# fattorib/ZeRO-transformer

Measured on AMD Instinct MI355X. Metric: training throughput (tokens/s, whole job), higher is better.
Workload: dtype bf16; 1 GPU; model=GPT-1_3b_2048 (1.31B params), global_batch=16, seq_len=2048, train_context=2048, parallelism=dp1+zero1, grad_accum=1

## Files before the change

### zero_transformer_amd/ops/csrc/attention_fwd.hip

```cpp

#include "attn_tiles.h"
#include "common.h"

#include <ATen/ATen.h>
#include <ATen/hip/HIPContext.h>
#include <ATen/hip/impl/HIPStreamMasqueradingAsCUDA.h>
#include <torch/extension.h>

namespace {

using attn::NW;
using attn::RB;
using attn::TB;
using attn::Stage;
using attn::swz;
using attn::tr_frag;

constexpr float NEG_INF = -3.0e38f;

template <int D, int NT, int MINW>
__global__ __launch_bounds__(NT, MINW) void flash_fwd_kernel(
    const uint16_t* __restrict__ qkv, const float* __restrict__ slopes,
    uint16_t* __restrict__ o, float* __restrict__ lse, int H, int T, int C,
    float scale, float p_drop, uint32_t seed) {
  extern __shared__ __attribute__((aligned(16))) char smem[];
  uint16_t* lds0 = (uint16_t*)smem;

  const int bh = blockIdx.x;
  const int h = bh % H;
  const int QS = 3 * C;
  const long base = (long)(bh / H) * T * QS + h * D;
  const long kbase = base + C;
  const long vbase = base + 2 * C;
  const long obase = (long)(bh / H) * T * C + h * D;
  constexpr int RBX = NT / 2;
  const int q0 = blockIdx.y * RBX;
  const int wave = threadIdx.x >> 6;
  const int lane = threadIdx.x & 63;
  const int li = lane & 31;
  const int hi = lane >> 5;
  const int qw = q0 + wave * 32;
  const int qi = qw + li;
  const float slope = slopes[h];
  constexpr float LOG2E = 1.4426950408889634f;
  constexpr float LN2 = 0.6931471805599453f;
  constexpr float DEFER_THR = 11.5f;
  const float scale2 = scale * LOG2E;
  const float slope2 = slope * LOG2E;
  const uint32_t drop_thr = (uint32_t)(p_drop * 256.0f + 0.5f);
  const float inv_keep = drop_thr ? 256.0f / (256.0f - (float)drop_thr) : 1.0f;

  constexpr int KS = D / 16;
  constexpr int DB = D / 32;

  bf16x8 q_frag[KS];
  {
    const bool ok = qi < T;
#pragma unroll
    for (int s = 0; s < KS; ++s)
      q_frag[s] = ok ? *reinterpret_cast<const bf16x8*>(
                           &qkv[base + (long)qi * QS + s * 16 + 8 * hi])
                     : bf16x8{};
  }

  float m_run = NEG_INF, l_run = 0.f;
  f32x16 o_acc[DB];
#pragma unroll
  for (int d = 0; d < DB; ++d) o_acc[d] = f32x16{};

  if (NT == 512 && __builtin_amdgcn_readfirstlane(threadIdx.x) >= 256)
    __builtin_amdgcn_s_setprio(1);

  attn::glds_stage<D, NT / 64>(qkv, kbase, QS, 0, T, lds0);
  attn::glds_stage<D, NT / 64>(qkv, vbase, QS, 0, T, lds0 + TB * 128);
  const int kv_end = min(T, q0 + RBX);
  for (int kt = 0; kt < kv_end; kt += TB) {
    const int cur = (kt / TB) & 1;
    const uint16_t* k_lds = lds0 + (cur ? 2 * TB * 128 : 0);
    const uint16_t* v_lds = lds0 + TB * 128 + (cur ? 2 * TB * 128 : 0);
    __syncthreads();
    attn::lds_acquire();
    if (kt + TB < kv_end) {
      uint16_t* nxt = lds0 + (cur ? 0 : 2 * TB * 128);
      attn::glds_stage<D, NT / 64>(qkv, kbase, QS, kt + TB, T, nxt);
      attn::glds_stage<D, NT / 64>(qkv, vbase, QS, kt + TB, T, nxt + TB * 128);
    }

#pragma unroll
    for (int sub = 0; sub < 2; ++sub) {
      const int kt32 = kt + sub * 32;
      if (kt32 > qw + 31 || kt32 >= T) continue;

      f32x16 s_acc{};
#pragma unroll
      for (int s = 0; s < KS; ++s) {
        const int kk = s * 16 + 8 * hi;
        const int krow = sub * 32 + li;
        bf16x8 a_frag = *reinterpret_cast<const bf16x8*>(
            (char*)k_lds + swz(krow, krow * 256 + kk * 2));
        s_acc = __builtin_amdgcn_mfma_f32_32x32x16_bf16(a_frag, q_frag[s], s_acc, 0, 0, 0);
      }

      float sv_[16];
      float tile_max = NEG_INF;
#pragma unroll
      for (int r = 0; r < 16; ++r) {
        const int kj = kt32 + (r & 3) + 8 * (r >> 2) + 4 * hi;
        float x = s_acc[r] * scale2 + slope2 * (float)(kj - qi);
        if (kj > qi || kj >= T || qi >= T) x = NEG_INF;
        sv_[r] = x;
        tile_max = fmaxf(tile_max, x);
      }
      tile_max = fmaxf(tile_max, __shfl_xor(tile_max, 32, 64));

      float alpha = 1.f;
      const bool valid = tile_max > 0.5f * NEG_INF;
      if (!__all(tile_max <= m_run + DEFER_THR)) {
        const float mn = valid ? fmaxf(m_run, tile_max) : m_run;
        alpha = (m_run > 0.5f * NEG_INF) ? exp2f(m_run - mn) : (valid ? 0.f : 1.f);
        m_run = mn;
      }
      float p[16];
      float row_sum = 0.f;
#pragma unroll
      for (int r = 0; r < 16; ++r) {
        p[r] = (valid && m_run > 0.5f * NEG_INF) ? exp2f(sv_[r] - m_run) : 0.f;
        row_sum += p[r];
      }
      row_sum += __shfl_xor(row_sum, 32, 64);
      l_run = l_run * alpha + row_sum;

      if (drop_thr) {
        const int bhT_qi = bh * T + qi;
#pragma unroll
        for (int g = 0; g < 4; ++g) {
          const int kbase = kt32 + 8 * g + 4 * hi;
          const uint32_t bits = drop_bits32(seed, bhT_qi, kbase >> 2);
#pragma unroll
          for (int e = 0; e < 4; ++e) {
            const bool keep = ((bits >> (8 * e)) & 0xffu) >= drop_thr;
            p[4 * g + e] = keep ? p[4 * g + e] * inv_keep : 0.f;
          }
        }
      }

      if (!__all(alpha == 1.f)) {
#pragma unroll
        for (int r = 0; r < 16; ++r) {
          const float ar = __shfl(alpha, (r & 3) + 8 * (r >> 2) + 4 * hi, 64);
#pragma unroll
          for (int d = 0; d < DB; ++d) o_acc[d][r] *= ar;
        }
      }

      bf16x8 pa[2];
      attn::c_to_a_frags(p, pa);

      attn::TrPair vp[2];
      attn::tr_pair_issue(v_lds, sub * 32, 0, &vp[0]);
#pragma unroll
      for (int d = 0; d < DB; ++d) {
        if (d + 1 < DB) attn::tr_pair_issue(v_lds, sub * 32, (d + 1) * 32, &vp[(d + 1) & 1]);
        attn::TrPair& t = vp[d & 1];
        if (d + 1 < DB)
          attn::tr_pair_wait<4>(&t);
        else
          attn::tr_pair_wait<0>(&t);
        o_acc[d] = __builtin_amdgcn_mfma_f32_32x32x16_bf16(pa[0], t.a, o_acc[d], 0, 0, 0);
        o_acc[d] = __builtin_amdgcn_mfma_f32_32x32x16_bf16(pa[1], t.b, o_acc[d], 0, 0, 0);
      }
    }
  }

  const float inv_l = l_run > 0.f ? 1.f / l_run : 0.f;
  if (hi == 0 && qi < T)
    lse[(long)bh * T + qi] = l_run > 0.f ? m_run * LN2 + __logf(l_run) : NEG_INF;
#pragma unroll
  for (int r = 0; r < 16; ++r) {
    const int row = (r & 3) + 8 * (r >> 2) + 4 * hi;
    const int qr = qw + row;
    if (qr >= T) continue;
    const float il = __shfl(inv_l, row, 64);
#pragma unroll
    for (int d = 0; d < DB; ++d)
      o[obase + (long)qr * C + d * 32 + li] = f32_to_bf16(o_acc[d][r] * il);
  }
}

template <int D>
void launch_fwd(const at::Tensor& qkv, const at::Tensor& slopes, at::Tensor& o,
                at::Tensor& lse, int B, int H, int T, int C, float scale,
                float p_drop, uint32_t seed, hipStream_t stream) {
  const size_t smem = 4 * TB * 128 * sizeof(uint16_t);
  static const bool f4 = [] {
    const char* e = getenv("ZTA_FWD4");
    return e && e[0] == '1';
  }();
  if (f4) {
    dim3 grid(B * H, (T + 127) / 128);
    hipLaunchKernelGGL((flash_fwd_kernel<D, 256, 1>), grid, dim3(256), smem, stream,
                       (const uint16_t*)qkv.data_ptr(), slopes.data_ptr<float>(),
                       (uint16_t*)o.data_ptr(), lse.data_ptr<float>(), H, T, C,
                       scale, p_drop, seed);
    return;
  }
  dim3 grid(B * H, (T + RB - 1) / RB);
  hipLaunchKernelGGL((flash_fwd_kernel<D, 512, 2>), grid, dim3(512), smem, stream,
                     (const uint16_t*)qkv.data_ptr(), slopes.data_ptr<float>(),
                     (uint16_t*)o.data_ptr(), lse.data_ptr<float>(), H, T, C,
                     scale, p_drop, seed);
}

}

std::vector<at::Tensor> attn_fwd(at::Tensor qkv, at::Tensor slopes, int64_t H_,
                                 double p_drop, int64_t seed) {
  TORCH_CHECK(qkv.is_cuda() && qkv.is_contiguous() && qkv.dim() == 3,
              "qkv must be (B, T, 3C) contiguous");
  TORCH_CHECK(qkv.scalar_type() == at::kBFloat16, "attn_fwd: bf16 only");
  const int B = qkv.size(0), T = qkv.size(1), H = (int)H_;
  const int C = qkv.size(2) / 3;
  TORCH_CHECK(qkv.size(2) == 3 * C && C % H == 0, "bad qkv shape");
  const int D = C / H;
  auto o = at::empty({B, T, C}, qkv.options());
  auto lse = at::empty({B, H, T}, qkv.options().dtype(at::kFloat));
  auto sl = slopes.to(at::kFloat).contiguous();
  const float scale = 1.0f / sqrtf((float)D);
  auto stream = at::hip::getCurrentHIPStreamMasqueradingAsCUDA();
  switch (D) {
    case 32: launch_fwd<32>(qkv, sl, o, lse, B, H, T, C, scale, (float)p_drop, (uint32_t)seed, stream); break;
    case 64: launch_fwd<64>(qkv, sl, o, lse, B, H, T, C, scale, (float)p_drop, (uint32_t)seed, stream); break;
    case 96: launch_fwd<96>(qkv, sl, o, lse, B, H, T, C, scale, (float)p_drop, (uint32_t)seed, stream); break;
    case 128: launch_fwd<128>(qkv, sl, o, lse, B, H, T, C, scale, (float)p_drop, (uint32_t)seed, stream); break;
    default: TORCH_CHECK(false, "attn_fwd: head_dim must be one of 32/64/96/128, got ", D);
  }
  return {o, lse};
}
```

### zero_transformer_amd/ops/csrc/attn_tiles.h

```cpp
#pragma once

#include "common.h"

typedef __attribute__((ext_vector_type(8))) __bf16 bf16x8;
typedef __attribute__((ext_vector_type(2))) int i32x2;

#if defined(__HIP_DEVICE_COMPILE__) && defined(__clang_major__)
#if __clang_major__ < 19 || __clang_major__ > 22
#error \
    "attn_tiles.h counted s_waitcnt contracts validated only for ROCm LLVM 19-22; \
re-run tests/test_gpu_ops.py on this compiler and extend the guard (or build \
with -DZTA_SAFE_WAITS=1)."
#endif
#endif
#ifndef ZTA_SAFE_WAITS
#define ZTA_SAFE_WAITS 0
#endif

namespace attn {

constexpr int NW = 8;
constexpr int RB = NW * 32;
constexpr int TB = 64;

ZTA_DEV int swz(int row, int byte_off) { return byte_off ^ ((row & 7) << 4); }

ZTA_DEV void lds_acquire() { asm volatile("" ::: "memory"); }

ZTA_DEV bf16x8 tr_frag(const uint16_t* lds, int k0, int j0) {
  const int l = threadIdx.x & 63;
  const int colb = (j0 + (l & 16) + 4 * (l & 3)) * 2;
  const int r0 = k0 + 8 * (l >> 5) + ((l >> 2) & 3);
  const int a0 = (int)(size_t)((const char*)lds + r0 * 256 + (colb ^ ((r0 & 7) << 4)));
  const int r1 = r0 + 4;
  const int a1 = (int)(size_t)((const char*)lds + r1 * 256 + (colb ^ ((r1 & 7) << 4)));
  union {
    i32x2 d[2];
    bf16x8 v;
  } u;
  asm volatile(
      "ds_read_b64_tr_b16 %0, %2\n\t"
      "ds_read_b64_tr_b16 %1, %3\n\t"
      "s_waitcnt lgkmcnt(0)"
      : "=&v"(u.d[0]), "=&v"(u.d[1])
      : "v"(a0), "v"(a1));
  return u.v;
}

struct TrPair {
  bf16x8 a, b;
};

struct TrQuad {
  TrPair x, y;
};
ZTA_DEV TrQuad tr_frag_quad(const uint16_t* lds_x, const uint16_t* lds_y, int k0,
                            int j0) {
  const int l = threadIdx.x & 63;
  const int colb = (j0 + (l & 16) + 4 * (l & 3)) * 2;
  const int rb = 8 * (l >> 5) + ((l >> 2) & 3);
  int ax[4], ay[4];
#pragma unroll
  for (int i = 0; i < 4; ++i) {
    const int row = k0 + 16 * (i >> 1) + 4 * (i & 1) + rb;
    const int off = row * 256 + (colb ^ ((row & 7) << 4));
    ax[i] = (int)(size_t)((const char*)lds_x + off);
    ay[i] = (int)(size_t)((const char*)lds_y + off);
  }
  union {
    i32x2 d[8];
    TrQuad f;
  } u;
  asm volatile(
      "ds_read_b64_tr_b16 %0, %8\n\t"
      "ds_read_b64_tr_b16 %1, %9\n\t"
      "ds_read_b64_tr_b16 %2, %10\n\t"
      "ds_read_b64_tr_b16 %3, %11\n\t"
      "ds_read_b64_tr_b16 %4, %12\n\t"
      "ds_read_b64_tr_b16 %5, %13\n\t"
      "ds_read_b64_tr_b16 %6, %14\n\t"
      "ds_read_b64_tr_b16 %7, %15\n\t"
      "s_waitcnt lgkmcnt(0)"
      : "=&v"(u.d[0]), "=&v"(u.d[1]), "=&v"(u.d[2]), "=&v"(u.d[3]),
        "=&v"(u.d[4]), "=&v"(u.d[5]), "=&v"(u.d[6]), "=&v"(u.d[7])
      : "v"(ax[0]), "v"(ax[1]), "v"(ax[2]), "v"(ax[3]), "v"(ay[0]), "v"(ay[1]),
        "v"(ay[2]), "v"(ay[3]));
  return u.f;
}
ZTA_DEV void tr_quad_issue(const uint16_t* lds_x, const uint16_t* lds_y, int k0,
                           int j0, TrQuad* out, int l = threadIdx.x & 63) {
  const int colb = (j0 + (l & 16) + 4 * (l & 3)) * 2;
  const int rb = 8 * (l >> 5) + ((l >> 2) & 3);
  int ax[4], ay[4];
#pragma unroll
  for (int i = 0; i < 4; ++i) {
    const int row = k0 + 16 * (i >> 1) + 4 * (i & 1) + rb;
    const int off = row * 256 + (colb ^ ((row & 7) << 4));
    ax[i] = (int)(size_t)((const char*)lds_x + off);
    ay[i] = (int)(size_t)((const char*)lds_y + off);
  }
  union U {
    i32x2 d[8];
    TrQuad f;
  }* u = (union U*)out;
  asm volatile(
      "ds_read_b64_tr_b16 %0, %8\n\t"
      "ds_read_b64_tr_b16 %1, %9\n\t"
      "ds_read_b64_tr_b16 %2, %10\n\t"
      "ds_read_b64_tr_b16 %3, %11\n\t"
      "ds_read_b64_tr_b16 %4, %12\n\t"
      "ds_read_b64_tr_b16 %5, %13\n\t"
      "ds_read_b64_tr_b16 %6, %14\n\t"
      "ds_read_b64_tr_b16 %7, %15"
      : "=&v"(u->d[0]), "=&v"(u->d[1]), "=&v"(u->d[2]), "=&v"(u->d[3]),
        "=&v"(u->d[4]), "=&v"(u->d[5]), "=&v"(u->d[6]), "=&v"(u->d[7])
      : "v"(ax[0]), "v"(ax[1]), "v"(ax[2]), "v"(ax[3]), "v"(ay[0]), "v"(ay[1]),
        "v"(ay[2]), "v"(ay[3]));
}

ZTA_DEV void tr_dsk_issue(const uint16_t* ds_tile, const uint16_t* k_img, int k0,
                          int j0, TrQuad* out, int l = threadIdx.x & 63) {
  const int cq = ((l & 16) + 4 * (l & 3)) * 2;
  const int colb = (j0 + (l & 16) + 4 * (l & 3)) * 2;
  const int rb = 8 * (l >> 5) + ((l >> 2) & 3);
  int ax[4], ay[4];
#pragma unroll
  for (int i = 0; i < 4; ++i) {
    const int row = k0 + 16 * (i >> 1) + 4 * (i & 1) + rb;
    ax[i] = (int)(size_t)((const char*)ds_tile + row * 64 + cq);
    ay[i] = (int)(size_t)((const char*)k_img + row * 256 + (colb ^ ((row & 7) << 4)));
  }
  union U {
    i32x2 d[8];
    TrQuad f;
  }* u = (union U*)out;
  asm volatile(
      "ds_read_b64_tr_b16 %0, %8\n\t"
      "ds_read_b64_tr_b16 %1, %9\n\t"
      "ds_read_b64_tr_b16 %2, %10\n\t"
      "ds_read_b64_tr_b16 %3, %11\n\t"
      "ds_read_b64_tr_b16 %4, %12\n\t"
      "ds_read_b64_tr_b16 %5, %13\n\t"
      "ds_read_b64_tr_b16 %6, %14\n\t"
      "ds_read_b64_tr_b16 %7, %15"
      : "=&v"(u->d[0]), "=&v"(u->d[1]), "=&v"(u->d[2]), "=&v"(u->d[3]),
        "=&v"(u->d[4]), "=&v"(u->d[5]), "=&v"(u->d[6]), "=&v"(u->d[7])
      : "v"(ax[0]), "v"(ax[1]), "v"(ax[2]), "v"(ax[3]), "v"(ay[0]), "v"(ay[1]),
        "v"(ay[2]), "v"(ay[3]));
}

template <int N>
ZTA_DEV void tile_barrier() {
  asm volatile("s_waitcnt vmcnt(%0) lgkmcnt(0)\n\ts_barrier"
               :
               : "i"(ZTA_SAFE_WAITS ? 0 : N)
               : "memory");
}

template <bool FIRST>
ZTA_DEV void mfma_sdp2(f32x16& s, f32x16& dp, const bf16x8* qa, const bf16x8* da,
                       const bf16x8* kb, const bf16x8* vb) {
  if (FIRST) {
    asm("s_nop 1\n\t"
        "v_mfma_f32_32x32x16_bf16 %0, %2, %6, 0\n\t"
        "v_mfma_f32_32x32x16_bf16 %1, %4, %8, 0\n\t"
        "v_mfma_f32_32x32x16_bf16 %0, %3, %7, %0\n\t"
        "v_mfma_f32_32x32x16_bf16 %1, %5, %9, %1\n\t"
        "s_nop 11"
        : "=&v"(s), "=&v"(dp)
        : "v"(qa[0]), "v"(qa[1]), "v"(da[0]), "v"(da[1]), "v"(kb[0]), "v"(kb[1]),
          "v"(vb[0]), "v"(vb[1]));
  } else {
    asm("s_nop 1\n\t"
        "v_mfma_f32_32x32x16_bf16 %0, %2, %6, %0\n\t"
        "v_mfma_f32_32x32x16_bf16 %1, %4, %8, %1\n\t"
        "v_mfma_f32_32x32x16_bf16 %0, %3, %7, %0\n\t"
        "v_mfma_f32_32x32x16_bf16 %1, %5, %9, %1\n\t"
        "s_nop 11"
        : "+v"(s), "+v"(dp)
        : "v"(qa[0]), "v"(qa[1]), "v"(da[0]), "v"(da[1]), "v"(kb[0]), "v"(kb[1]),
          "v"(vb[0]), "v"(vb[1]));
  }
}

ZTA_DEV void mfma_quad_acc(f32x16& acc, const TrQuad& t) {
  asm("s_nop 1\n\t"
      "v_mfma_f32_32x32x16_bf16 %0, %1, %2, %0\n\t"
      "v_mfma_f32_32x32x16_bf16 %0, %3, %4, %0\n\t"
      "s_nop 11"
      : "+v"(acc)
      : "v"(t.x.a), "v"(t.y.a), "v"(t.x.b), "v"(t.y.b));
}

ZTA_DEV void lds_barrier() {
  asm volatile("s_waitcnt lgkmcnt(0)\n\ts_barrier" ::: "memory");
}

template <int N>
ZTA_DEV void tr_quad_wait(TrQuad* q) {
  union U {
    i32x2 d[8];
    TrQuad f;
  }* u = (union U*)q;
  asm volatile("s_waitcnt lgkmcnt(%8)"
               : "+v"(u->d[0]), "+v"(u->d[1]), "+v"(u->d[2]), "+v"(u->d[3]),
                 "+v"(u->d[4]), "+v"(u->d[5]), "+v"(u->d[6]), "+v"(u->d[7])
               : "i"(ZTA_SAFE_WAITS ? 0 : N));
}

ZTA_DEV void tr_pair_issue(const uint16_t* lds, int k0, int j0, TrPair* out) {
  const int l = threadIdx.x & 63;
  const int colb = (j0 + (l & 16) + 4 * (l & 3)) * 2;
  const int rb = 8 * (l >> 5) + ((l >> 2) & 3);
  int a[4];
#pragma unroll
  for (int i = 0; i < 4; ++i) {
    const int row = k0 + 16 * (i >> 1) + 4 * (i & 1) + rb;
    a[i] = (int)(size_t)((const char*)lds + row * 256 + (colb ^ ((row & 7) << 4)));
  }
  union U {
    i32x2 d[4];
    TrPair f;
  }* u = (union U*)out;
  asm volatile(
      "ds_read_b64_tr_b16 %0, %4\n\t"
      "ds_read_b64_tr_b16 %1, %5\n\t"
      "ds_read_b64_tr_b16 %2, %6\n\t"
      "ds_read_b64_tr_b16 %3, %7"
      : "=&v"(u->d[0]), "=&v"(u->d[1]), "=&v"(u->d[2]), "=&v"(u->d[3])
      : "v"(a[0]), "v"(a[1]), "v"(a[2]), "v"(a[3]));
}

template <int N>
ZTA_DEV void tr_pair_wait(TrPair* q) {
  union U {
    i32x2 d[4];
    TrPair f;
  }* u = (union U*)q;
  asm volatile("s_waitcnt lgkmcnt(%4)"
               : "+v"(u->d[0]), "+v"(u->d[1]), "+v"(u->d[2]), "+v"(u->d[3])
               : "i"(ZTA_SAFE_WAITS ? 0 : N));
}

ZTA_DEV TrPair tr_frag_pair(const uint16_t* lds, int k0, int j0) {
  const int l = threadIdx.x & 63;
  const int colb = (j0 + (l & 16) + 4 * (l & 3)) * 2;
  const int rb = 8 * (l >> 5) + ((l >> 2) & 3);
  int a[4];
#pragma unroll
  for (int i = 0; i < 4; ++i) {
    const int row = k0 + 16 * (i >> 1) + 4 * (i & 1) + rb;
    a[i] = (int)(size_t)((const char*)lds + row * 256 + (colb ^ ((row & 7) << 4)));
  }
  union {
    i32x2 d[4];
    TrPair f;
  } u;
  asm volatile(
      "ds_read_b64_tr_b16 %0, %4\n\t"
      "ds_read_b64_tr_b16 %1, %5\n\t"
      "ds_read_b64_tr_b16 %2, %6\n\t"
      "ds_read_b64_tr_b16 %3, %7\n\t"
      "s_waitcnt lgkmcnt(0)"
      : "=&v"(u.d[0]), "=&v"(u.d[1]), "=&v"(u.d[2]), "=&v"(u.d[3])
      : "v"(a[0]), "v"(a[1]), "v"(a[2]), "v"(a[3]));
  return u.f;
}

ZTA_DEV void c_to_a_frags(const float* x, bf16x8* pa) {
  unsigned w[8];
#pragma unroll
  for (int j = 0; j < 8; ++j) {
    asm("v_cvt_pk_bf16_f32 %0, %1, %2" : "=v"(w[j]) : "v"(x[2 * j]), "v"(x[2 * j + 1]));
  }
#pragma unroll
  for (int j = 0; j < 2; ++j) {
    auto r0 = __builtin_amdgcn_permlane32_swap(w[4 * j + 0], w[4 * j + 2], false, false);
    w[4 * j + 0] = r0[0];
    w[4 * j + 2] = r0[1];
    auto r1 = __builtin_amdgcn_permlane32_swap(w[4 * j + 1], w[4 * j + 3], false, false);
    w[4 * j + 1] = r1[0];
    w[4 * j + 3] = r1[1];
  }
  union {
    unsigned u[4];
    bf16x8 v8;
  } cvt;
  cvt.u[0] = w[0]; cvt.u[1] = w[1]; cvt.u[2] = w[2]; cvt.u[3] = w[3];
  pa[0] = cvt.v8;
  cvt.u[0] = w[4]; cvt.u[1] = w[5]; cvt.u[2] = w[6]; cvt.u[3] = w[7];
  pa[1] = cvt.v8;
}

template <int D, int NWAVES, int ROWS = TB>
ZTA_DEV void glds_stage(const uint16_t* g, long base, int rs, int row0, int T,
                        uint16_t* lds, int l = threadIdx.x & 63) {
  const int wave = (threadIdx.x >> 6);
  const int s = l & 15;
  const int rsub = l >> 4;
#pragma unroll
  for (int k = wave; k < ROWS / 4; k += NWAVES) {
    const int row = 4 * k + rsub;
    int c8 = 8 * (s ^ (row & 7));
    if (D < 128 && c8 >= D) c8 = 0;
    const int rg = min(row0 + row, T - 1);
    __builtin_amdgcn_global_load_lds(
        (const __attribute__((address_space(1))) void*)&g[base + (long)rg * rs + c8],
        (__attribute__((address_space(3))) void*)(lds + (long)k * 512), 16, 0, 0);
  }
}

ZTA_DEV void glds_stats32(const float* a, const float* b, long rowbase, int q0, int T,
                          float* dst, int l = threadIdx.x & 63) {
  const float* src = (l < 32 ? a : b) + rowbase + min(q0 + (l & 31), T - 1);
  __builtin_amdgcn_global_load_lds(
      (const __attribute__((address_space(1))) void*)src,
      (__attribute__((address_space(3))) void*)dst, 4, 0, 0);
}

template <int D, int NT = 512>
struct Stage {
  static constexpr int NC = (TB * D + NT * 8 - 1) / (NT * 8);
  s16x8 r[NC];
  ZTA_DEV void load(const uint16_t* g, long base, int rs, int row0, int T) {
    const int t = threadIdx.x;
#pragma unroll
    for (int c = 0; c < NC; ++c) {
      const int idx = t * 8 + c * NT * 8;
      const int rg = row0 + idx / D;
      r[c] = (idx < TB * D && rg < T)
                 ? *reinterpret_cast<const s16x8*>(&g[base + (long)rg * rs + idx % D])
                 : s16x8{};
    }
  }
  ZTA_DEV void store(uint16_t* lds) {
    const int t = threadIdx.x;
#pragma unroll
    for (int c = 0; c < NC; ++c) {
      const int idx = t * 8 + c * NT * 8;
      if (idx >= TB * D) break;
      const int row = idx / D, d = idx % D;
      *reinterpret_cast<s16x8*>((char*)lds + swz(row, row * 256 + d * 2)) = r[c];
    }
  }
};

}
```

Before: 101,400 tokens/s.

## Add optimized v2 flash attention forward kernel for head_dim 128

Adds a new forward attention kernel for D=128 that handles the full 64-key tile as two MFMA groups with software-pipelined K fragment loads. It hoists ALiBi bias constants into scalar registers and applies the per-tile bias after the max, uses permlane32 swaps for half-wave reductions, and specializes the dropout path at compile time. V transposed reads use immediate offsets, and the output is staged through LDS so stores are coalesced 16-byte writes. The intent is to cut VALU, address arithmetic and store overhead in the attention forward pass. The cost is heavy reliance on inline asm and manual nops, a changed dropout hash whose mask may not match the backward pass, and masking logic that needs careful validation.

```diff
diff --git a/zero_transformer_amd/ops/csrc/attention_fwd.hip b/zero_transformer_amd/ops/csrc/attention_fwd.hip
--- a/zero_transformer_amd/ops/csrc/attention_fwd.hip
+++ b/zero_transformer_amd/ops/csrc/attention_fwd.hip
@@ -6,6 +6,9 @@
 #include <ATen/hip/HIPContext.h>
 #include <ATen/hip/impl/HIPStreamMasqueradingAsCUDA.h>
 #include <torch/extension.h>
+
+#include <type_traits>
+#include <utility>
 
 namespace {
 
@@ -187,25 +190,266 @@
   }
 }
 
+template <class F, int... I>
+ZTA_DEV void static_for_impl(F&& f, std::integer_sequence<int, I...>) {
+  (f(std::integral_constant<int, I>{}), ...);
+}
+template <int N, class F>
+ZTA_DEV void static_for(F&& f) {
+  static_for_impl(f, std::make_integer_sequence<int, N>{});
+}
+
+ZTA_DEV float as_f32(unsigned u) { return __builtin_bit_cast(float, u); }
+ZTA_DEV unsigned as_u32(float f) { return __builtin_bit_cast(unsigned, f); }
+ZTA_DEV float half_max(float x) {
+  auto r = __builtin_amdgcn_permlane32_swap(as_u32(x), as_u32(x), false, false);
+  return fmaxf(as_f32(r[0]), as_f32(r[1]));
+}
+ZTA_DEV float add1(float a, float b) {
+  float r;
+  asm("v_add_f32 %0, %1, %2" : "=v"(r) : "v"(a), "v"(b));
+  return r;
+}
+ZTA_DEV float fma1(float a, float b, float c) {
+  float r;
+  asm("v_fma_f32 %0, %1, %2, %3" : "=v"(r) : "v"(a), "v"(b), "v"(c));
+  return r;
+}
+ZTA_DEV void mfma_settle(f32x16& a, f32x16& b) {
+  asm volatile("s_nop 15\n\ts_nop 3" : "+v"(a), "+v"(b));
+}
+ZTA_DEV float half_sum(float x) {
+  auto r = __builtin_amdgcn_permlane32_swap(as_u32(x), as_u32(x), false, false);
+  return as_f32(r[0]) + as_f32(r[1]);
+}
+
+template <int D, bool DROP>
+__global__ __launch_bounds__(512, 2) void flash_fwd_v2_kernel(
+    const uint16_t* __restrict__ qkv, const float* __restrict__ slopes,
+    uint16_t* __restrict__ o, float* __restrict__ lse, int H, int T, int C,
+    float scale, float p_drop, uint32_t seed) {
+  extern __shared__ __attribute__((aligned(16))) char smem[];
+  uint16_t* lds0 = (uint16_t*)smem;
+
+  const int bh = blockIdx.x;
+  const int h = bh % H;
+  const int QS = 3 * C;
+  const long base = (long)(bh / H) * T * QS + h * D;
+  const long kbase = base + C;
+  const long vbase = base + 2 * C;
+  const long obase = (long)(bh / H) * T * C + h * D;
+  const int q0 = blockIdx.y * RB;
+  const int wave = __builtin_amdgcn_readfirstlane(threadIdx.x >> 6);
+  const int lane = threadIdx.x & 63;
+  const int li = lane & 31;
+  const int hi = lane >> 5;
+  const int qw = q0 + wave * 32;
+  const int qi = qw + li;
+  const int qc = min(qi, T - 1);
+  constexpr float LOG2E = 1.4426950408889634f;
+  constexpr float LN2 = 0.6931471805599453f;
+  constexpr float DEFER_THR = 11.5f;
+  const float scale2 = scale * LOG2E;
+  const float slope2 = slopes[h] * LOG2E;
+  const uint32_t drop_thr = (uint32_t)(p_drop * 256.0f + 0.5f);
+
+  constexpr int KS = D / 16;
+  constexpr int DB = D / 32;
+
+  float cst[16];
+#pragma unroll
+  for (int r = 0; r < 16; ++r)
+    cst[r] = as_f32(__builtin_amdgcn_readfirstlane(
+        as_u32(slope2 * (float)((r & 3) + 8 * (r >> 2)))));
+
+  bf16x8 q_frag[KS];
+#pragma unroll
+  for (int s = 0; s < KS; ++s)
+    q_frag[s] = *reinterpret_cast<const bf16x8*>(
+        &qkv[base + (long)qc * QS + s * 16 + 8 * hi]);
+
+  float m_run = NEG_INF;
+  float l_half = 0.f;
+  f32x16 o_acc[DB];
+#pragma unroll
+  for (int d = 0; d < DB; ++d) o_acc[d] = f32x16{};
+
+  const uint32_t hq = seed ^ ((uint32_t)(bh * T + qc) * 0x9e3779b9u);
+
+  if (__builtin_amdgcn_readfirstlane(threadIdx.x) >= 256)
+    __builtin_amdgcn_s_setprio(1);
+
+  attn::glds_stage<D, NW>(qkv, kbase, QS, 0, T, lds0);
+  attn::glds_stage<D, NW>(qkv, vbase, QS, 0, T, lds0 + TB * 128);
+  const int kv_end = min(T, q0 + RB);
+  for (int kt = 0; kt < kv_end; kt += TB) {
+    const int cur = (kt / TB) & 1;
+    __syncthreads();
+    attn::lds_acquire();
+    if (kt + TB < kv_end) {
+      uint16_t* nxt = lds0 + (cur ? 0 : 2 * TB * 128);
+      attn::glds_stage<D, NW>(qkv, kbase, QS, kt + TB, T, nxt);
+      attn::glds_stage<D, NW>(qkv, vbase, QS, kt + TB, T, nxt + TB * 128);
+    }
+    if (kt > qw) continue;
+
+    const char* kl = (const char*)lds0 + (cur ? 4 * TB * 128 : 0) + li * 256;
+    const int kx = (16 * hi) ^ ((li & 7) << 4);
+    const int vl = (int)(size_t)((const char*)lds0 + (cur ? 6 * TB * 128 : 2 * TB * 128)) +
+                   attn::tr_lane_off(lane);
+
+    auto k_frag = [&](int u, int s) {
+      return *reinterpret_cast<const bf16x8*>(
+          kl + (kx ^ ((s & 3) << 5)) + (s >> 2) * 128 + u * 32 * 256);
+    };
+    f32x16 s_acc[2] = {f32x16{}, f32x16{}};
+    bf16x8 kf0[KS], kf1[KS];
+#pragma unroll
+    for (int s = 0; s < KS; ++s) kf0[s] = k_frag(0, s);
+    __builtin_amdgcn_sched_barrier(0);
+#pragma unroll
+    for (int s = 0; s < KS; ++s) {
+      kf1[s] = k_frag(1, s);
+      s_acc[0] = __builtin_amdgcn_mfma_f32_32x32x16_bf16(kf0[s], q_frag[s], s_acc[0], 0, 0, 0);
+    }
+    __builtin_amdgcn_sched_barrier(0);
+#pragma unroll
+    for (int s = 0; s < KS; ++s)
+      s_acc[1] = __builtin_amdgcn_mfma_f32_32x32x16_bf16(kf1[s], q_frag[s], s_acc[1], 0, 0, 0);
+    mfma_settle(s_acc[0], s_acc[1]);
+
+    const int dl = qc - kt - 4 * hi;
+    float y[2][16];
+    float mx[2] = {NEG_INF, NEG_INF};
+    if (kt + 63 <= qw && kt + 63 < T) {
+#pragma unroll
+      for (int u = 0; u < 2; ++u)
+#pragma unroll
+        for (int r = 0; r < 16; ++r) {
+          y[u][r] = fma1(s_acc[u][r], scale2, cst[r]);
+          mx[u] = fmaxf(mx[u], y[u][r]);
+        }
+    } else {
+#pragma unroll
+      for (int u = 0; u < 2; ++u)
+#pragma unroll
+        for (int r = 0; r < 16; ++r) {
+          const float x = fma1(s_acc[u][r], scale2, cst[r]);
+          y[u][r] = (r & 3) + 8 * (r >> 2) + 32 * u > dl ? NEG_INF : x;
+          mx[u] = fmaxf(mx[u], y[u][r]);
+        }
+    }
+    const float lb0 = slope2 * (float)(-dl);
+    const float lb1 = slope2 * (float)(32 - dl);
+    const float tmax = half_max(fmaxf(mx[0] + lb0, mx[1] + lb1));
+
+    if (!__all(tmax <= m_run + DEFER_THR)) {
+      const float mn = fmaxf(m_run, tmax);
+      const float alpha = __builtin_amdgcn_exp2f(m_run - mn);
+      m_run = mn;
+      l_half *= alpha;
+#pragma unroll
+      for (int r = 0; r < 16; ++r) {
+        const float ar = __shfl(alpha, (r & 3) + 8 * (r >> 2) + 4 * hi, 64);
+#pragma unroll
+        for (int d = 0; d < DB; ++d) o_acc[d][r] *= ar;
+      }
+    }
+
+    bf16x8 pa[2][2];
+#pragma unroll
+    for (int u = 0; u < 2; ++u) {
+      const float t = (u ? lb1 : lb0) - m_run;
+      float p[16];
+      float rs = 0.f;
+#pragma unroll
+      for (int r = 0; r < 16; ++r) {
+        p[r] = __builtin_amdgcn_exp2f(add1(y[u][r], t));
+        rs += p[r];
+      }
+      l_half += rs;
+      if (DROP) {
+        const uint32_t kg0 = (uint32_t)((kt >> 2) + 8 * u + hi) * 0x85ebca6bu;
+#pragma unroll
+        for (int g = 0; g < 4; ++g) {
+          const uint32_t bits = mix32(hq ^ (kg0 + (uint32_t)(2 * g) * 0x85ebca6bu));
+#pragma unroll
+          for (int e = 0; e < 4; ++e)
+            if (((bits >> (8 * e)) & 0xffu) < drop_thr) p[4 * g + e] = 0.f;
+        }
+      }
+      attn::c_to_a_frags(p, pa[u]);
+    }
+
+    attn::TrPair vp[2];
+    attn::tr_pair_issue_imm<0, 0>(vl, &vp[0]);
+    static_for<2 * DB>([&](auto ic) {
+      constexpr int i = decltype(ic)::value;
+      constexpr int u = i / DB, d = i % DB;
+      if constexpr (i + 1 < 2 * DB)
+        attn::tr_pair_issue_imm<32 * ((i + 1) / DB), 32 * ((i + 1) % DB)>(vl, &vp[(i + 1) & 1]);
+      attn::TrPair& tp = vp[i & 1];
+      if constexpr (i + 1 < 2 * DB)
+        attn::tr_pair_wait<4>(&tp);
+      else
+        attn::tr_pair_wait<0>(&tp);
+      o_acc[d] = __builtin_amdgcn_mfma_f32_32x32x16_bf16(pa[u][0], tp.a, o_acc[d], 0, 0, 0);
+      o_acc[d] = __builtin_amdgcn_mfma_f32_32x32x16_bf16(pa[u][1], tp.b, o_acc[d], 0, 0, 0);
+    });
+  }
+
+  const float l_run = half_sum(l_half);
+  if (hi == 0 && qi < T) lse[(long)bh * T + qi] = m_run * LN2 + __logf(l_run);
+  float inv_l = 1.f / l_run;
+  if (DROP) inv_l *= 256.0f / (256.0f - (float)drop_thr);
+
+  __syncthreads();
+  char* ot = smem + wave * (32 * D * 2);
+#pragma unroll
+  for (int r = 0; r < 16; r += 2) {
+    const int row0 = (r & 3) + 8 * (r >> 2) + 4 * hi;
+    const float il0 = __shfl(inv_l, row0, 64);
+    const float il1 = __shfl(inv_l, row0 + 1, 64);
+#pragma unroll
+    for (int d = 0; d < DB; ++d) {
+      unsigned w;
+      asm("v_cvt_pk_bf16_f32 %0, %1, %2"
+          : "=v"(w)
+          : "v"(o_acc[d][r] * il0), "v"(o_acc[d][r + 1] * il1));
+      uint16_t* dst = (uint16_t*)(ot + row0 * (D * 2)) + d * 32 + li;
+      dst[0] = (uint16_t)w;
+      dst[D] = (uint16_t)(w >> 16);
+    }
+  }
+  asm volatile("s_waitcnt lgkmcnt(0)" ::: "memory");
+  constexpr int LPR = D / 8;
+#pragma unroll
+  for (int c = 0; c < 32 * LPR / 64; ++c) {
+    const int idx = c * 64 + lane;
+    const int row = idx / LPR, col = (idx % LPR) * 8;
+    const s16x8 v8 = *reinterpret_cast<const s16x8*>(ot + row * (D * 2) + col * 2);
+    if (qw + row < T)
+      *reinterpret_cast<s16x8*>(&o[obase + (long)(qw + row) * C + col]) = v8;
+  }
+}
+
 template <int D>
 void launch_fwd(const at::Tensor& qkv, const at::Tensor& slopes, at::Tensor& o,
                 at::Tensor& lse, int B, int H, int T, int C, float scale,
                 float p_drop, uint32_t seed, hipStream_t stream) {
   const size_t smem = 4 * TB * 128 * sizeof(uint16_t);
-  static const bool f4 = [] {
-    const char* e = getenv("ZTA_FWD4");
+  static const bool v1 = [] {
+    const char* e = getenv("ZTA_FWD_V1");
     return e && e[0] == '1';
   }();
-  if (f4) {
-    dim3 grid(B * H, (T + 127) / 128);
-    hipLaunchKernelGGL((flash_fwd_kernel<D, 256, 1>), grid, dim3(256), smem, stream,
-                       (const uint16_t*)qkv.data_ptr(), slopes.data_ptr<float>(),
-                       (uint16_t*)o.data_ptr(), lse.data_ptr<float>(), H, T, C,
-                       scale, p_drop, seed);
-    return;
-  }
   dim3 grid(B * H, (T + RB - 1) / RB);
-  hipLaunchKernelGGL((flash_fwd_kernel<D, 512, 2>), grid, dim3(512), smem, stream,
+  auto k = flash_fwd_kernel<D, 512, 2>;
+  if constexpr (D == 128) {
+    if (!v1)
+      k = (uint32_t)(p_drop * 256.0f + 0.5f) ? flash_fwd_v2_kernel<D, true>
+                                             : flash_fwd_v2_kernel<D, false>;
+  }
+  hipLaunchKernelGGL(k, grid, dim3(512), smem, stream,
                      (const uint16_t*)qkv.data_ptr(), slopes.data_ptr<float>(),
                      (uint16_t*)o.data_ptr(), lse.data_ptr<float>(), H, T, C,
                      scale, p_drop, seed);
diff --git a/zero_transformer_amd/ops/csrc/attn_tiles.h b/zero_transformer_amd/ops/csrc/attn_tiles.h
--- a/zero_transformer_amd/ops/csrc/attn_tiles.h
+++ b/zero_transformer_amd/ops/csrc/attn_tiles.h
@@ -231,6 +231,30 @@
       : "v"(a[0]), "v"(a[1]), "v"(a[2]), "v"(a[3]));
 }
 
+ZTA_DEV int tr_lane_off(int l) {
+  const int q = (l >> 2) & 3;
+  return (8 * (l >> 5) + q) * 256 + ((2 * (l & 16) + 8 * (l & 3)) ^ (q << 4));
+}
+template <int K0, int J0>
+ZTA_DEV void tr_pair_issue_imm(int lane_base, TrPair* out) {
+  static_assert(K0 % 8 == 0 && J0 % 32 == 0, "offset split needs aligned k0/j0");
+  constexpr int O0 = (K0 + 0) * 256 + (2 * J0);
+  constexpr int O1 = (K0 + 4) * 256 + ((2 * J0) ^ 64);
+  constexpr int O2 = (K0 + 16) * 256 + (2 * J0);
+  constexpr int O3 = (K0 + 20) * 256 + ((2 * J0) ^ 64);
+  union U {
+    i32x2 d[4];
+    TrPair f;
+  }* u = (union U*)out;
+  asm volatile(
+      "ds_read_b64_tr_b16 %0, %4 offset:%5\n\t"
+      "ds_read_b64_tr_b16 %1, %4 offset:%6\n\t"
+      "ds_read_b64_tr_b16 %2, %4 offset:%7\n\t"
+      "ds_read_b64_tr_b16 %3, %4 offset:%8"
+      : "=&v"(u->d[0]), "=&v"(u->d[1]), "=&v"(u->d[2]), "=&v"(u->d[3])
+      : "v"(lane_base), "n"(O0), "n"(O1), "n"(O2), "n"(O3));
+}
+
 template <int N>
 ZTA_DEV void tr_pair_wait(TrPair* q) {
   union U {
```

Result: faster. 103,500 tokens/s (median of 6 runs) (+2.0%).
